# AnteMarusic/Accelerating-Genomics

Measured on AMD Instinct MI355X. Metric: Smith-Waterman affine-gap score-only GCUPS (config 2: 65536 pairs 150x150 per GPU), higher is better.
Workload: dtype int16x2 lanes, int32 scores; 1 GPU; BASELINE config 2: 65536 SW pairs 150x150 per GPU, iid ACGT + 25% related, newline sentinel aligned as the reference does; pairs_per_gpu=65536, len=150, cells_counted_per_pair=22500, parallelism=pairs sharded per GPU, no collective

## Files before the change

accelerating-genomics_amd/api.py:

```python
from __future__ import annotations

import ctypes as C
import os
import subprocess

import numpy as np

_HERE = os.path.dirname(os.path.abspath(__file__))
TUNING_KNOBS = ("AGX_SW_KERNEL", "AGX_SW_TAIL_BETA", "AGX_SW_MAX_C", "AGX_SW_FORCE_C", "AGX_SW_MAX_CLASSES", "AGX_SW_WAVES_PER_CLASS",
                "AGX_SW_SORT_WAVES", "AGX_SW_ONE_LAUNCH", "AGX_SW_DNA", "AGX_SW_RISE", "AGX_SW_PERIOD", "AGX_PHMM_PLAIN_CELL", "AGX_TRACE_CREATE", "AGX_HOST_THREADS", "AGX_FANOUT", "AGX_PHMM_TAB_BUDGET", "AGX_PHMM_MAX_C",
                "AGX_PHMM_FORCE_C", "AGX_PHMM_TAIL_BETA", "AGX_PHMM_MAX_CLASSES", "AGX_PHMM_NO_LUT", "AGX_TRACE_POOL", "AGX_NO_STREAM_PRIO", "AGX_SW_I32_CLASSIC", "AGX_SW_PIECE_MB", "AGX_SW_PIECE_MIN_PAIRS", "AGX_PHMM_NO_ROWS", "AGX_PHMM_NO_TRAINS", "AGX_PHMM_LUT_ONE_LOOP", "AGX_SW_HOST_PLAN", "AGX_PHMM_NO_RING", "AGX_TRACE_CIGAR")
_DEFAULT_LIB = "libagx_tuning.so" if any(k in os.environ for k in TUNING_KNOBS) else "libagx.so"
LIB_PATH = os.environ.get("AGX_LIB_PATH", os.path.join(_HERE, _DEFAULT_LIB))

OK, E_ARG, E_NODEVICE, E_HIP, E_NOMEM, E_SYMBOL, E_LIMIT, E_IO, E_INTERNAL = 0, -1, -2, -3, -4, -5, -6, -7, -8
SW_ALIGN_ENDS, SW_ALIGN_SPANS = 1, 2
SW_ALIGN_MAX_QUERY_LEN, SW_ALIGN_MAX_TARGET_LEN = 2560, 65535
SW_MODE_LOCAL, SW_MODE_GLOBAL, SW_MODE_FIT, SW_MODE_EXTEND, SW_MODE_EXTEND_QUERY = 0, 1, 2, 3, 4
SwHit = np.dtype([("score", np.int32), ("a_begin", np.int32), ("a_end", np.int32), ("b_begin", np.int32), ("b_end", np.int32)])
SwStat = np.dtype([("matches", np.int32), ("pairs", np.int32)])
SW_STATS_MAX_QUERY_LEN = 1792
SW_CIGAR_MAX_QUERY_LEN = 2048
CIGAR_INS, CIGAR_DEL, CIGAR_EQ, CIGAR_DIFF = 1, 2, 7, 8
_CIGAR_CHARS = {CIGAR_INS: "I", CIGAR_DEL: "D", CIGAR_EQ: "=", CIGAR_DIFF: "X"}
OPT_SW_KERNEL = 1
OPT_SW_PLANNER = 2
SW_PLANNER_AUTO, SW_PLANNER_HOST, SW_PLANNER_DEVICE = 0, 1, 2
OPT_PHMM_TRAINS = 3
OPT_SW_TRACE_BYTES = 4
PHMM_TRAINS_AUTO, PHMM_TRAINS_OFF, PHMM_TRAINS_ON = 0, 1, 2
SW_KERNEL_AUTO, SW_KERNEL_INT32, SW_KERNEL_PACKED_SIGNED, SW_KERNEL_PACKED_BIASED = 0, 1, 2, 3
PHMM_F64, PHMM_F64_FMA, PHMM_F32, PHMM_F32_FMA = 0, 1, 2, 3
PHMM_GATK_PRIOR = 0x100

SYMBOLS = [
    "agx_version", "agx_last_error", "agx_device_count", "agx_device_name", "agx_ctx_create", "agx_ctx_destroy", "agx_ctx_device",
    "agx_ctx_stream", "agx_ctx_set_stream", "agx_ctx_sync", "agx_ctx_set_option", "agx_warmup_devices", "agx_host_alloc", "agx_host_free",
    "agx_ctx_timer_start", "agx_ctx_timer_stop", "agx_ctx_timer_mark", "agx_ctx_timer_elapsed",
    "agx_sw_batch_create", "agx_sw_batch_create_scored", "agx_sw_batch_create_matrix", "agx_sw_batch_launch", "agx_sw_batch_scores", "agx_sw_batch_bind_scores", "agx_sw_batch_info", "agx_sw_batch_destroy",
    "agx_sw_batch_create_align", "agx_sw_batch_hits", "agx_sw_align", "agx_sw_batch_create_align_mode", "agx_sw_align_mode",
    "agx_sw_batch_create_align_matrix", "agx_sw_align_matrix",
    "agx_sw_batch_create_align_stats", "agx_sw_batch_stats", "agx_sw_align_stats",
    "agx_sw_batch_create_align_cigar", "agx_sw_batch_cigars", "agx_sw_batch_cigar_info", "agx_sw_align_cigar",
# ... 561 lines not shown
```

accelerating-genomics_amd/csrc/agx_sw.cpp:

```cpp
#include "agx_sw.h"

#include <algorithm>
#include <cmath>
#include <memory>
#include <mutex>
#include <thread>

#include "agx_internal.h"
#include "agx_parallel.h"

namespace {

struct Tiling {
    int cls;
    int G;
};

bool positive(long n) { return n > 0; }
bool at_least_4(long n) { return n >= 4; }
inline double tail_beta_override() { static const double v = agx_knob_real(agx_tune("AGX_SW_TAIL_BETA"), -1.0); return v; }
int max_cols_per_lane() { static const int v = (int)agx_knob_int(agx_tune("AGX_SW_MAX_C"), AGX_SW_MAX_COLS_PER_LANE, at_least_4); return v; }
int force_cols_per_lane() { static const int v = (int)agx_knob_int(agx_tune("AGX_SW_FORCE_C"), 0); return v; }
int max_classes_override() { static const int v = (int)agx_knob_int(agx_tune("AGX_SW_MAX_CLASSES"), 0, positive); return v; }
int tuned_kernel()
// ... 152 lines not shown
struct agx_sw_batch {
    agx_ctx *ctx = nullptr;
    int family = 0;
    int align = 0;
    int mode = 0;
    int stats = 0;
    DevBuf lstat;
    PinBuf lstat_stage;
    int cigar = 0;
    std::vector<uint64_t> tr_goff;
    std::vector<SwWalkRec> tr_walk;
    uint64_t tr_dwords = 0, tr_slot_words = 0;
    DevBuf goff, walkrec;
    uint32_t *trace_p = nullptr;
    bool cig_valid = false;
    std::vector<agx_sw_hit> cig_hits;
    std::vector<uint64_t> cig_off;
    std::vector<uint32_t> cig_ops;
    agx_sw_cigar_info cig_info{};
    std::vector<int64_t> fix_pair;
    std::vector<int32_t> fix_score;
    agx_sw_scoring scoring{};
    DevBuf ends;
    PinBuf ends_stage;
    std::vector<uint8_t> seq;
    std::vector<uint64_t> seq_off;
    std::vector<uint32_t> seq_len;
    SwParams prm{};
    int64_t n_pairs = 0;
    DevBuf img, groups, waves, scores;
    DevBuf table;
    int rising = 0;
    bool wide = false;
    PinBuf out_stage;
    bool matrix = false;
    agx_sw_matrix mat{};
    std::vector<ClassLaunch> launches;
    agx_sw_info info{};
    struct SwPending *pending = nullptr;
    bool file_order = false;
    int32_t *bound = nullptr;
};

namespace {
int create_batch(agx_ctx *ctx, const agx_sw_scoring *scoring, const agx_sw_matrix *matrix, const uint8_t *bases,
                 const uint64_t *off, const uint32_t *len, int64_t n_pairs, agx_sw_batch **out, bool defer = false, int align = 0, int mode = 0,
                 int stats = 0, int cigar = 0);
int finish_create(agx_sw_batch *b);
void drop_pending(agx_sw_batch *b);
}

extern "C" {

void agx_sw_batch_destroy(agx_sw_batch *b)
{
    if (!b) return;
    if (b->ctx) (void)hipSetDevice(b->ctx->device);
    drop_pending(b);
    b->img.release();
    b->groups.release();
    b->waves.release();
    b->scores.release();
    b->table.release();
    b->out_stage.release();
    b->ends.release();
    b->ends_stage.release();
// ... 1014 lines not shown
                b->tr_goff[q.group0 + g] = at;
                SwWalkRec &r = b->tr_walk[pp.pair];
                r.goff = at;
                r.x_dw = x_dw[q.first + g];
                r.y_dw = y_dw[q.first + g];
                r.ca = pp.lx();
                r.cb = pp.ly;
                r.G = (uint16_t)q.G;
                r.C = (uint16_t)C;
                at += sw_trace_dwords(q.G, pp.ly, C);
            }
        b->tr_dwords = at;
        uint64_t words = 0;
        for (SwWalkRec &r : b->tr_walk) {
            r.slot = words;
            words += (uint64_t)r.ca + r.cb;
        }
        b->tr_slot_words = words;
    }
    t_records = agx_now_ms();

    }
    b->launches = launches;
    if (family == 2 && rising == 4) {
        int period = 4;
        for (int k = 0; k < kSwNumClasses; ++k)
            if ((launched_classes >> k & 1u) && kSwClasses[k] <= kSwPackedMaxShort / 64) period = std::max(period, sw_pk2_period(kSwClasses[k]));
        bool wide = period > 4 && (int64_t)bias + ((int64_t)longest_short + 1) * sc.match - prm.gf +
                                          ((int64_t)longest_long + 65 + period) * -(int64_t)prm.ge < 0x7c00;
        if (const char *e = agx_tune("AGX_SW_PERIOD")) wide = wide && !(e[0] == '4' && !e[1]);
        b->wide = wide;
        if (wide && ctx) agx_sw_pk2w_preload();
        if (trace) fprintf(stderr, "[agx_sw_batch_create] class period %d of %d\n", wide ? period : 4, period);
    }
    b->info.n_pairs = n_pairs;
    b->info.cells = cells;
    b->info.padded_cells = padded;
    b->info.input_bytes = (int64_t)(img_dw * 4 + groups_bytes + waves_bytes);
    b->info.n_launches = (int32_t)launches.size();
    b->info.n_waves = (int32_t)n_waves_total;
    b->info.planned_on_device = device_plan ? 1 : 0;
    if (!ctx) {
        if (trace)
            fprintf(stderr, "[agx_sw_batch_create, plan only] %lld pairs: pass A %.2f ms | tiling %.2f, sort %.2f, waves %.2f, records %.2f\n",
                    (long long)n_pairs, t_pass_a - t_begin, t_plan - t_pass_a, t_sort - t_plan, t_waves - t_sort, t_records - t_waves);
        *out = b;
        b = nullptr;
        done.ok = true;
        return AGX_OK;
    }

    if (uploader.joinable()) uploader.join();
    if (up_rc) {
        agx_set_error("%s", up_err);
        return up_rc;
    }
    const double t_joined = agx_now_ms();
    rc = b->img.alloc(ctx, std::max<size_t>(img_dw, 4) * 4);
    if (!rc && !device_plan) rc = b->groups.alloc(ctx, groups_bytes);
    if (!rc && !device_plan) rc = b->waves.alloc(ctx, waves_bytes);
    if (!rc && matrix) rc = b->table.alloc(ctx, table.size() * sizeof(int16_t));
    if (!rc) rc = b->scores.alloc(ctx, ((size_t)n_pairs + 1) * sizeof(int32_t));
    if (!rc) rc = b->out_stage.alloc(ctx, ((size_t)n_pairs + 1) * sizeof(int32_t));
    if (!rc && align) rc = b->ends.alloc(ctx, ((size_t)n_pairs + 1) * sizeof(uint32_t));
    if (!rc && align) rc = b->ends_stage.alloc(ctx, ((size_t)n_pairs + 1) * sizeof(uint32_t));
    if (!rc && stats == 2) rc = b->lstat.alloc(ctx, ((size_t)n_pairs + 1) * sizeof(uint32_t));
// ... 122 lines not shown
            r = agx_sw_trace_launch_class(cl.C, prm, img, (const SwGroup *)b->groups.p, wv, cl.n_waves, scores, (uint32_t *)b->ends.p, b->trace_p,
                                          (const uint64_t *)b->goff.p, st);
        else if (b->stats == 2 && b->family == 5 && b->matrix)
            r = agx_sw_anch_mat_stats_launch_class(cl.C, anch_capture, anch_flags, prm, img, (const SwGroup *)b->groups.p, wv, cl.n_waves, scores,
                                                   (uint32_t *)b->ends.p, lstat, (const int16_t *)b->table.p, st);
        else if (b->stats == 2 && b->family == 5)
            r = agx_sw_anch_stats_launch_class(cl.C, anch_capture, anch_flags, prm, img, (const SwGroup *)b->groups.p, wv, cl.n_waves, scores,
                                               (uint32_t *)b->ends.p, lstat, st);
        else if (b->stats == 2 && b->matrix)
            r = agx_sw_loc_mat_stats_launch_class(cl.C, prm, img, (const SwGroup *)b->groups.p, wv, cl.n_waves, scores, (uint32_t *)b->ends.p, lstat,
                                                  (const int16_t *)b->table.p, st);
        else if (b->stats == 2)
            r = agx_sw_loc_stats_launch_class(cl.C, prm, img, (const SwGroup *)b->groups.p, wv, cl.n_waves, scores, (uint32_t *)b->ends.p, lstat, st);
        else if (b->family == 5 && b->matrix)
            r = agx_sw_anch_mat_launch_class(cl.C, anch_capture, anch_flags, prm, img, (const SwGroup *)b->groups.p, wv, cl.n_waves, scores,
                                             (uint32_t *)b->ends.p, (const int16_t *)b->table.p, st);
        else if (b->family == 5)
            r = agx_sw_anch_launch_class(cl.C, anch_capture, anch_flags, prm, img, (const SwGroup *)b->groups.p, wv, cl.n_waves, scores,
                                         (uint32_t *)b->ends.p, st);
        else if (b->align && b->matrix)
            r = agx_sw_loc_mat_launch_class(cl.C, prm, img, (const SwGroup *)b->groups.p, wv, cl.n_waves, scores, (uint32_t *)b->ends.p,
                                            (const int16_t *)b->table.p, st);
        else if (b->align)
            r = agx_sw_loc_launch_class(cl.C, prm, img, (const SwGroup *)b->groups.p, wv, cl.n_waves, scores, (uint32_t *)b->ends.p, st);
        else if (b->matrix)
            r = agx_sw_mat_launch_class(cl.C, prm, img, (const SwGroup *)b->groups.p, wv, cl.n_waves, scores,
                                        (const int16_t *)b->table.p, st);
        else if (b->family == 3)
            r = cl.C == 0 ? agx_sw_i32d_launch_any(prm, img, (const SwGroup2 *)b->groups.p, wv, cl.n_waves, scores, st)
                          : agx_sw_i32d_launch_class(cl.C, prm, img, (const SwGroup2 *)b->groups.p, wv, cl.n_waves, scores, st);
        else if (b->family == 2 && cl.C == 0)
            r = agx_sw_pk2_launch_any(b->rising, b->wide, prm, img, (const SwGroup2 *)b->groups.p, wv, cl.n_waves, scores, st);
        else if (b->family == 2)
            r = agx_sw_pk2_launch_class(cl.C, b->rising, b->wide, prm, img, (const SwGroup2 *)b->groups.p, wv, cl.n_waves, scores, st);
        else if (b->family == 1)
            r = agx_sw_pk_launch_class(cl.C, prm, img, (const SwGroup2 *)b->groups.p, wv, cl.n_waves, scores, st);
        else
            r = (cl.C > 40 ? agx_sw_wide_launch_class : agx_sw_launch_class)(cl.C, prm, img, (const SwGroup *)b->groups.p, wv,
                                                                             cl.n_waves, scores, st);
        if (r) {
            agx_set_error("sw_fill<%d> launch failed: %s", cl.C, hipGetErrorString(hipGetLastError()));
            return AGX_E_HIP;
        }
    }
    return fan.end();
}

int agx_sw_batch_scores(agx_sw_batch *b, int32_t *scores)
{
    if (!b || (!scores && b->n_pairs)) {
        agx_set_error("agx_sw_batch_scores: null argument");
        return AGX_E_ARG;
    }
    if (!b->ctx) {
        agx_set_error("this batch was planned without a context (no device): it has no scores");
        return AGX_E_NODEVICE;
    }
    int rc = agx_bind(b->ctx);
    if (rc) return rc;
    if (b->pending) {
        rc = finish_create(b);
        if (rc) return rc;
    }
    if (b->n_pairs == 0) {
        AGX_HIP(hipStreamSynchronize(b->ctx->stream));
        return AGX_OK;
    }
// ... 838 lines not shown
```

accelerating-genomics_amd/csrc/agx_sw.h:

```cpp
#pragma once
#include <hip/hip_runtime.h>

#include <algorithm>
#include <cstdint>

#include "../../include/agx.h"

struct SwGroup {
    uint32_t x_dw;
    uint32_t y_dw;
    uint32_t lx_ly;
    uint32_t out;
};

struct SwParams {
    int32_t ge;
    int32_t gf;
    int32_t hd;
    int32_t delta;
    int32_t shift;
    uint32_t ge2, gf2, hd2, delta2;
    uint32_t age2, agf2, bias2;
    uint32_t n_out;
};
// ... 7 lines not shown

struct SwWave {
    uint32_t first_group;
    uint16_t n_groups;
    uint16_t G;
    uint32_t steps;
    uint32_t reserved;
};

#define AGX_SW_FOR_EACH_CLASS(X) \
    X(4) X(6) X(8) X(10) X(12) X(14) X(16) X(18) X(20) X(22) X(24) X(26) X(28) X(30) X(32) X(34) X(36) X(38) X(40)
#define AGX_SW_FOR_EACH_WIDE_CLASS(X) X(80) X(120) X(160)
static const int kSwClasses[] = {4, 6, 8, 10, 12, 14, 16, 18, 20, 22, 24, 26, 28, 30, 32, 34, 36, 38, 40, 80, 120, 160};
static const int kSwPackedMaxShort = 64 * 40;
static const int kSwNumClasses = sizeof(kSwClasses) / sizeof(kSwClasses[0]);
static const double kSwClassCost[] = {1.373, 1.250, 1.178, 1.138, 1.112, 1.080, 1.051, 1.033, 1.025, 1.022, 1.014, 1.014, 1.011, 1.007, 1.007, 1.004, 1.004, 1.004, 1.000, 1.6, 2.2, 4.0};
static const double kSwPkClassCost[] = {1.543, 1.358, 1.278, 1.210, 1.173, 1.136, 1.111, 1.086, 1.068, 1.037, 1.025, 1.025, 1.019, 1.012, 1.006, 1.006, 1.006, 1.000, 1.000, 0, 0, 0};
static const double kSwPk2ClassCost[] = {1.851, 1.581, 1.450, 1.367, 1.318, 1.263, 1.196, 1.184, 1.145, 1.097, 1.095, 1.056, 1.049, 1.053, 1.025, 1.023, 1.022, 1.016, 1.000, 0, 0, 0};

static const double kSwI32dClassCost[] = {1.373, 1.250, 1.178, 1.138, 1.112, 1.080, 1.051, 1.033, 1.025, 1.022, 1.014, 1.014, 1.011, 1.007, 1.007, 1.004, 1.004, 1.004, 1.000, 0, 0, 0};

constexpr int kSwMatDim = 33;
int agx_sw_mat_launch_class(int cols_per_lane, const SwParams &prm, const uint32_t *img, const SwGroup *groups,
                            const SwWave *waves, uint32_t n_waves, int32_t *scores, const int16_t *table, hipStream_t s);
int agx_sw_pack_launch(bool matrix, int slots, const uint8_t *raw, const uint64_t *off, uint64_t base, const void *groups,
                       uint32_t n_groups, uint32_t n_pairs, uint32_t *img, const uint8_t *code, uint32_t *flag, int n_cu,
                       hipStream_t s);
int agx_sw_pack_dna_launch(const uint8_t *raw, const uint64_t *off, uint64_t base, void *groups, void *waves, uint32_t n_waves,
                           uint32_t n_pairs, uint32_t *img, uint32_t *flag, int n_cu, hipStream_t s);
int agx_sw_pk_launch_class(int cols_per_lane, const SwParams &prm, const uint32_t *img, const SwGroup2 *groups,
                           const SwWave *waves, uint32_t n_waves, int32_t *scores, hipStream_t s);
#define AGX_SW_PK2_KEEP_NARROW(C) (false)
constexpr int sw_pk2_period(int C) { return C >= 14 && !AGX_SW_PK2_KEEP_NARROW(C) ? C / 2 : 4; }
int agx_sw_pk2_launch_class(int cols_per_lane, int rising, bool wide, const SwParams &prm, const uint32_t *img, const SwGroup2 *groups,
                            const SwWave *waves, uint32_t n_waves, int32_t *scores, hipStream_t s);
int agx_sw_pk2w_launch_class(int cols_per_lane, const SwParams &prm, const uint32_t *img, const SwGroup2 *groups, const SwWave *waves,
                             uint32_t n_waves, int32_t *scores, hipStream_t s);
int agx_sw_pk2w_launch_any(const SwParams &prm, const uint32_t *img, const SwGroup2 *groups, const SwWave *waves, uint32_t n_waves,
                           int32_t *scores, hipStream_t s);
void agx_sw_pk2w_preload();
void agx_sw_pk2_preload();
void agx_sw_pack_preload();
void agx_sw_i32_preload();
int agx_sw_pk2_launch_any(int rising, bool wide, const SwParams &prm, const uint32_t *img, const SwGroup2 *groups, const SwWave *waves,
                          uint32_t n_waves, int32_t *scores, hipStream_t s);
int agx_sw_i32d_launch_any(const SwParams &prm, const uint32_t *img, const SwGroup2 *groups, const SwWave *waves, uint32_t n_waves, int32_t *scores,
                           hipStream_t s);
int agx_sw_i32d_launch_class(int cols_per_lane, const SwParams &prm, const uint32_t *img, const SwGroup2 *groups, const SwWave *waves,
                             uint32_t n_waves, int32_t *scores, hipStream_t s);
void agx_sw_i32d_preload();
int agx_sw_launch_class(int cols_per_lane, const SwParams &prm, const uint32_t *img, const SwGroup *groups,
                        const SwWave *waves, uint32_t n_waves, int32_t *scores, hipStream_t s);
int agx_sw_wide_launch_class(int cols_per_lane, const SwParams &prm, const uint32_t *img, const SwGroup *groups,
                             const SwWave *waves, uint32_t n_waves, int32_t *scores, hipStream_t s);
constexpr int kSwLocColBits = 12;
int agx_sw_loc_launch_class(int cols_per_lane, const SwParams &prm, const uint32_t *img, const SwGroup *groups, const SwWave *waves,
                            uint32_t n_waves, int32_t *scores, uint32_t *ends, hipStream_t s);
void agx_sw_loc_preload();
int agx_sw_anch_launch_class(int cols_per_lane, int capture, int flags, const SwParams &prm, const uint32_t *img, const SwGroup *groups,
                             const SwWave *waves, uint32_t n_waves, int32_t *scores, uint32_t *ends, hipStream_t s);
void agx_sw_anch_preload();
int agx_sw_loc_mat_launch_class(int cols_per_lane, const SwParams &prm, const uint32_t *img, const SwGroup *groups, const SwWave *waves,
                                uint32_t n_waves, int32_t *scores, uint32_t *ends, const int16_t *table, hipStream_t s);
void agx_sw_loc_mat_preload();
int agx_sw_anch_mat_launch_class(int cols_per_lane, int capture, int flags, const SwParams &prm, const uint32_t *img, const SwGroup *groups,
                                 const SwWave *waves, uint32_t n_waves, int32_t *scores, uint32_t *ends, const int16_t *table, hipStream_t s);
void agx_sw_anch_mat_preload();
#define AGX_SW_FOR_EACH_STATS_CLASS(X) X(4) X(6) X(8) X(10) X(12) X(14) X(16) X(18) X(20) X(22) X(24) X(26) X(28)
// ... 69 lines not shown
```

accelerating-genomics_amd/csrc/agx_sw_pk2_kernel.hip:

```cpp
#include "agx_sw_pk2_kernel.inc"

namespace {

template <int C, int KC>
__global__ void __launch_bounds__(256) sw_fill_pk2(const SwParams prm, const uint32_t *__restrict__ img,
                                                   const SwGroup2 *__restrict__ groups,
                                                   const SwWave *__restrict__ waves, uint32_t n_waves,
                                                   int32_t *__restrict__ scores)
{
    const uint32_t wave = __builtin_amdgcn_readfirstlane(blockIdx.x * 4u + (threadIdx.x >> 6));
    if (wave >= n_waves) return;
    pk2_body<C, KC>(prm, img, groups, waves[wave], scores);
}

template <int KC>
__global__ void __launch_bounds__(256) sw_fill_pk2_any(const SwParams prm, const uint32_t *__restrict__ img,
                                                       const SwGroup2 *__restrict__ groups,
                                                       const SwWave *__restrict__ waves, uint32_t n_waves,
                                                       int32_t *__restrict__ scores)
{
    const uint32_t wave = __builtin_amdgcn_readfirstlane(blockIdx.x * 4u + (threadIdx.x >> 6));
    if (wave >= n_waves) return;
    const SwWave w = waves[wave];
    switch (__builtin_amdgcn_readfirstlane(w.reserved) & 0xffffu) {
// ... 1 lines not shown
    case CC: pk2_body<CC, KC>(prm, img, groups, w, scores); break;
        AGX_SW_FOR_EACH_CLASS(AGX_SW_CASE)
#undef AGX_SW_CASE
    default: break;
    }
}

template <int C, int KC>
int launch(const SwParams &prm, const uint32_t *img, const SwGroup2 *groups, const SwWave *waves, uint32_t n_waves,
           int32_t *scores, hipStream_t s)
{
    const uint32_t blocks = (n_waves + 3) / 4;
    hipLaunchKernelGGL((sw_fill_pk2<C, KC>), dim3(blocks), dim3(256), 0, s, prm, img, groups, waves, n_waves, scores);
    return hipGetLastError() == hipSuccess ? 0 : -1;
}

}

int agx_sw_pk2_launch_any(int rising, bool wide, const SwParams &prm, const uint32_t *img, const SwGroup2 *groups, const SwWave *waves,
                          uint32_t n_waves, int32_t *scores, hipStream_t s)
{
    if (n_waves == 0) return 0;
    if (rising == 4 && wide) return agx_sw_pk2w_launch_any(prm, img, groups, waves, n_waves, scores, s);
    const uint32_t blocks = (n_waves + 3) / 4;
    if (rising == 4)
        hipLaunchKernelGGL(sw_fill_pk2_any<4>, dim3(blocks), dim3(256), 0, s, prm, img, groups, waves, n_waves, scores);
    else if (rising)
        hipLaunchKernelGGL(sw_fill_pk2_any<1>, dim3(blocks), dim3(256), 0, s, prm, img, groups, waves, n_waves, scores);
    else
        hipLaunchKernelGGL(sw_fill_pk2_any<0>, dim3(blocks), dim3(256), 0, s, prm, img, groups, waves, n_waves, scores);
    return hipGetLastError() == hipSuccess ? 0 : -1;
}

int agx_sw_pk2_launch_class(int cols_per_lane, int rising, bool wide, const SwParams &prm, const uint32_t *img, const SwGroup2 *groups,
                            const SwWave *waves, uint32_t n_waves, int32_t *scores, hipStream_t s)
{
    if (n_waves == 0) return 0;
    if (rising == 4 && wide && sw_pk2_period(cols_per_lane) > 4)
        return agx_sw_pk2w_launch_class(cols_per_lane, prm, img, groups, waves, n_waves, scores, s);
    switch (cols_per_lane) {
#define AGX_SW_CASE(CC) \
    case CC: return rising == 4 ? launch<CC, 4>(prm, img, groups, waves, n_waves, scores, s) : rising ? launch<CC, 1>(prm, img, groups, waves, n_waves, scores, s) : launch<CC, 0>(prm, img, groups, waves, n_waves, scores, s);
        AGX_SW_FOR_EACH_CLASS(AGX_SW_CASE)
#undef AGX_SW_CASE
    default: return -2;
    }
}

void agx_sw_pk2_preload()
{
    hipFuncAttributes a;
    (void)hipFuncGetAttributes(&a, reinterpret_cast<const void *>(&sw_fill_pk2_any<4>));
}
```

accelerating-genomics_amd/csrc/agx_sw_pk2_kernel.inc:

```
#include "agx_sw.h"
#include <type_traits>

namespace {

typedef unsigned short u16x2 __attribute__((ext_vector_type(2)));

__device__ __forceinline__ u16x2 as_v(uint32_t v) { return __builtin_bit_cast(u16x2, v); }
__device__ __forceinline__ uint32_t as_u(u16x2 v) { return __builtin_bit_cast(uint32_t, v); }
__device__ __forceinline__ uint32_t umax2(uint32_t a, uint32_t b) { return as_u(__builtin_elementwise_max(as_v(a), as_v(b))); }
__device__ __forceinline__ uint32_t umin2(uint32_t a, uint32_t b) { return as_u(__builtin_elementwise_min(as_v(a), as_v(b))); }
typedef _Float16 f16x2 __attribute__((ext_vector_type(2)));
__device__ __forceinline__ uint32_t umax3(uint32_t a, uint32_t b, uint32_t c)
{
    const f16x2 x = __builtin_bit_cast(f16x2, a), y = __builtin_bit_cast(f16x2, b), z = __builtin_bit_cast(f16x2, c);
    return __builtin_bit_cast(uint32_t, __builtin_elementwise_maximum(__builtin_elementwise_maximum(x, y), z));
}
__device__ __forceinline__ uint32_t in_vgpr(uint32_t s)
{
    uint32_t r;
    asm volatile("v_mov_b32 %0, %1" : "=v"(r) : "s"(s));
    return r;
}

#define AGX_DPP_TAKE " wave_shr:1 row_mask:0xf bank_mask:0xf bound_ctrl:0\n"
// ... 7 lines not shown
        : "=&v"(zl), "=&v"(fl), "+v"(ta), "+v"(tb), "=&v"(ma), "=&v"(mb)                                                     \
        : "v"(rowsA), "v"(rowsB), "v"(kv), "s"(start_mask), "v"(z_last), "v"(f_last), "v"(z0v)                               \
        : "vcc")

template <int K>
__device__ __forceinline__ void fast_head(uint32_t &zl, uint32_t &fl, uint32_t &ta, uint32_t &tb, uint32_t rowsA, uint32_t rowsB,
                                          uint32_t kv, uint64_t start_mask, uint32_t z_last, uint32_t f_last, uint32_t z0v)
{
    uint32_t ma, mb;
    if constexpr (K == 1)
        AGX_FAST_HEAD("BYTE_1");
    else if constexpr (K == 2)
        AGX_FAST_HEAD("BYTE_2");
    else if constexpr (K == 3)
        AGX_FAST_HEAD("BYTE_3");
    else
        AGX_FAST_HEAD("BYTE_0");
}

__device__ __forceinline__ void bytes_head(uint32_t &zl, uint32_t &fl, uint32_t &yc, uint32_t rowsA, uint32_t rowsB, uint32_t sel,
                                           uint32_t sh_sym, uint64_t start_mask, uint32_t z_last, uint32_t f_last, uint32_t z0v)
{
    uint32_t fresh;
    asm("v_perm_b32 %3, %5, %4, %6\n"
        "v_lshlrev_b32 %3, %7, %3\n"
        "s_mov_b64 vcc, %8\n"
        "v_cndmask_b32_dpp %0, %9, %11, vcc" AGX_DPP_TAKE "v_cndmask_b32_dpp %1, %10, %11, vcc" AGX_DPP_TAKE
        "v_cndmask_b32_dpp %2, %2, %3, vcc" AGX_DPP_TAKE
        : "=&v"(zl), "=&v"(fl), "+v"(yc), "=&v"(fresh)
        : "v"(rowsA), "v"(rowsB), "s"(sel), "v"(sh_sym), "s"(start_mask), "v"(z_last), "v"(f_last), "v"(z0v)
        : "vcc");
}

template <int C, bool FAST, int KC, bool WIDE = false>
__device__ __forceinline__ void pk2_fill(const SwParams &prm, const uint32_t *__restrict__ img, const SwGroup2 &g, const SwWave &w,
                                         int32_t *__restrict__ scores, int lane, int G, int gl, bool active, bool start, bool feeder)
{
    constexpr int XW = (C + 3) / 4;
    constexpr bool RISE = KC > 0;
    constexpr int NK = KC > 1 ? (WIDE ? C / 2 : KC) : 1;
    constexpr int kEnd = KC > 1 ? (C - 1) % NK : 0;
    constexpr int NM = KC > 1 ? NK + 3 : NK;
    const uint32_t sh_sym = prm.shift;
    const uint32_t col_pad = 0x100u << sh_sym;
    const uint32_t ge = in_vgpr(prm.age2), gf = in_vgpr(RISE ? prm.agf2 - prm.age2 : prm.agf2);
    const uint32_t hd = in_vgpr(FAST ? prm.hd2 - prm.delta2 : prm.hd2);
    const uint32_t bias = prm.bias2, delta = prm.delta2;
    const uint32_t z0 = prm.bias2 - prm.agf2;
    const uint32_t hd0 = in_vgpr((FAST ? prm.hd2 - prm.delta2 : prm.hd2) + (RISE ? prm.age2 : 0u));
    const uint32_t hdw = in_vgpr((FAST ? prm.hd2 - prm.delta2 : prm.hd2) + prm.age2 - (uint32_t)NK * prm.age2);
    const uint32_t ge_wrap = in_vgpr((uint32_t)NK * prm.age2), c_end = in_vgpr((uint32_t)kEnd * prm.age2);
    const uint32_t hdf = KC > 1 && kEnd > 0 ? in_vgpr((FAST ? prm.hd2 - prm.delta2 : prm.hd2) + prm.age2 - (uint32_t)kEnd * prm.age2) : hd0;
    const uint32_t ge4 = in_vgpr(4u * prm.age2);
    uint32_t zb = (RISE ? z0 + prm.age2 : z0) + (uint32_t)kEnd * prm.age2;
    constexpr bool FQ = WIDE && KC > 1;
    constexpr int NF = FQ ? NM : NK;
    uint32_t floorv[NF];
#pragma unroll
    for (int k = 0; k < NF; ++k) floorv[k] = (RISE ? bias + prm.age2 : bias) + (uint32_t)k * prm.age2;
    const uint32_t z_init = RISE ? z0 + prm.age2 : z0;
    const uint32_t kv = in_vgpr((prm.delta2 & 0xffu) << 24);
    const uint64_t start_mask = __ballot(start);
    const uint32_t lx_mask = FAST ? 0xfffu : 0x7fffu;
    const int lxA = (int)(g.lx_ly[0] & lx_mask), lxB = (int)(g.lx_ly[1] & lx_mask);
    const int lyA = (int)(g.lx_ly[0] >> 16), lyB = (int)(g.lx_ly[1] >> 16);

    const uint32_t no_row = FAST ? 0x1f1f1f1fu : 0u;
    const uint32_t *ybA = lyA > 0 ? img + g.y_dw[0] : img, *ybB = lyB > 0 ? img + g.y_dw[1] : img;
    const uint32_t lastA = lyA > 0 ? (uint32_t)((lyA + 3) >> 2) - 1u : 0u, lastB = lyB > 0 ? (uint32_t)((lyB + 3) >> 2) - 1u : 0u;
    const int nqA = feeder ? (lyA + 3) >> 2 : 0, nqB = feeder ? (lyB + 3) >> 2 : 0;
    auto loadA = [&](int q) -> uint32_t { return ybA[min((uint32_t)q, lastA)]; };
    auto loadB = [&](int q) -> uint32_t { return ybB[min((uint32_t)q, lastB)]; };
    auto row_selA = [&](int q, uint32_t v) -> uint32_t { return q < nqA ? v : no_row; };
    auto row_selB = [&](int q, uint32_t v) -> uint32_t { return q < nqB ? v : no_row; };

    uint32_t xq[C];
    constexpr int PF = C < 8 ? 2 : 1;
    uint32_t nextA[PF], nextB[PF];
    {
        const uint32_t o = (uint32_t)gl * C, d0 = o >> 2, sh = o & 3u;
        const uint32_t fillA = (FAST && !(active && g.x_dw[0])) ? 0x0c0c0c0cu : 0u;
        const uint32_t fillB = (FAST && !(active && g.x_dw[1])) ? 0x0c0c0c0cu : 0u;
        uint32_t ra[XW + 1], rb[XW + 1];
#pragma unroll
        for (int k = 0; k <= XW; ++k) {
            ra[k] = img[g.x_dw[0] + d0 + k];
            rb[k] = img[g.x_dw[1] + d0 + k];
        }
#pragma unroll
// ... 35 lines not shown
        z[j] = z_init + (uint32_t)(j % NK) * prm.age2;
        e[j] = bias + (uint32_t)(j % NK) * prm.age2;
    }
    uint32_t z_last = z_init + (uint32_t)kEnd * prm.age2, f_last = z_last, diag_in = z0 + (uint32_t)kEnd * prm.age2;
    uint32_t best[NM];
#pragma unroll
    for (int k = 0; k < NM; ++k) best[k] = z_init + (uint32_t)(KC > 1 ? k + 1 : k) * prm.age2;
    uint32_t yc = 0;
    uint32_t ta = 0, tb = 0;

    const bool last = active && gl == G - 1;
    const bool nlA = FAST && last && ((g.lx_ly[0] >> 13) & 1u), nlB = FAST && last && ((g.lx_ly[1] >> 13) & 1u);
    const int capA_t = (nlA && lxA > 0 && lyA > 0) ? lyA + G - 2 : -1, capB_t = (nlB && lxB > 0 && lyB > 0) ? lyB + G - 2 : -1;
    uint32_t cornerA = z_init + (uint32_t)kEnd * prm.age2, cornerB = cornerA;

    const int steps = (int)w.steps;
    uint32_t rowsA = 0, rowsB = 0;
    int t = 0;

    auto take_max = [&](auto sc) __attribute__((always_inline)) {
        constexpr int S = decltype(sc)::value;
#pragma unroll
        for (int k = 0; k < NK; ++k) {
#pragma unroll
            for (int j = k; j < C; j += 2 * NK) {
                if (j + NK < C)
                    best[S + k] = umax3(best[S + k], z[j], z[j + NK]);
                else
                    best[S + k] = umax2(best[S + k], z[j]);
            }
        }
    };

    auto step = [&](auto kc, auto sc, auto cc) __attribute__((always_inline)) {
        constexpr int K = decltype(kc)::value;
        constexpr int S = decltype(sc)::value;
        constexpr bool CAP = decltype(cc)::value;
        uint32_t zl, fl;
        if constexpr (FAST)
            fast_head<K>(zl, fl, ta, tb, rowsA, rowsB, kv, start_mask, z_last, f_last, zb);
        else
            bytes_head(zl, fl, yc, rowsA, rowsB, 0x0c040c00u + 0x00010001u * K, sh_sym, start_mask, z_last, f_last, zb);
        if constexpr (KC > 1 && S > 0 && S < 4)
            take_max(std::integral_constant<int, S - 1>{});
        else if constexpr (KC <= 1 && RISE)
            best[0] += ge;
        uint32_t zd = diag_in;
        diag_in = zl;
        uint32_t zleft = zl, f = fl;
#pragma unroll
        for (int j = 0; j < C; ++j) {
            const bool wrap = KC > 1 && j > 0 && j % NK == 0;
            const uint32_t up = z[j];
            uint32_t ev;
            if constexpr (RISE) {
                ev = umax3(up, e[j], floorv[(FQ && S < 4 ? S : 0) + j % NK]);
                f = umax2(zleft, f);
                if (KC == 1 && j > 0) f -= ge;
                if (KC > 1 && kEnd > 0 && j == 0) f -= c_end;
                if (wrap) f -= ge_wrap;
            } else {
                ev = umax3(up, e[j] - ge, bias);
                f = umax2(zleft, f - ge);
            }
            const uint32_t hdc = KC > 1 ? (wrap ? hdw : j ? hd0 : hdf) : (j ? hd : hd0);
            uint32_t u;
            if constexpr (FAST)
                u = (zd + hdc) + __builtin_amdgcn_perm(tb, ta, xq[j]);
            else
                u = (zd + hdc) - umin2(xq[j] ^ yc, delta);
            const uint32_t v = umax3(ev, f, u);
            const uint32_t zn = v - gf;
            e[j] = ev;
            z[j] = zn;
            zd = up;
            zleft = zn;
        }
        if constexpr (KC <= 1) {
#pragma unroll
            for (int j = 0; j < C; j += 2) best[0] = umax3(best[0], z[j], z[j + 1]);
        } else if constexpr (S >= 3)
            take_max(std::integral_constant<int, S == 3 ? 3 : 0>{});
        if constexpr (FAST && CAP) {
            cornerA = t == capA_t ? zleft : cornerA;
            cornerB = t == capB_t ? zleft : cornerB;
        }
        z_last = zleft;
        f_last = f;
        if constexpr (RISE) {
            if constexpr (!FQ || S == 4) {
#pragma unroll
                for (int k = 0; k < NF; ++k) floorv[k] += prm.age2;
            }
            zb += prm.age2;
        }
        ++t;
    };

    auto rise4 = [&]() __attribute__((always_inline)) {
        if constexpr (KC > 1) {
#pragma unroll
            for (int m = 0; m < NM; ++m) best[m] += ge4;
        }
        if constexpr (FQ) {
#pragma unroll
            for (int m = 0; m < NF; ++m) floorv[m] += 4u * prm.age2;
        }
    };
    auto quad_of_steps = [&](auto cc) __attribute__((always_inline)) {
        step(std::integral_constant<int, 0>{}, std::integral_constant<int, 0>{}, cc);
        step(std::integral_constant<int, 1>{}, std::integral_constant<int, 1>{}, cc);
        step(std::integral_constant<int, 2>{}, std::integral_constant<int, 2>{}, cc);
        step(std::integral_constant<int, 3>{}, std::integral_constant<int, 3>{}, cc);
        rise4();
    };
    auto take = [&](int q, int r) __attribute__((always_inline)) {
        rowsA = row_selA(q, nextA[r]);
        rowsB = row_selB(q, nextB[r]);
        nextA[r] = loadA(q + PF);
        nextB[r] = loadB(q + PF);
        if constexpr (WIDE) __builtin_amdgcn_sched_barrier(0);
    };
    const int quads = steps >> 2;
    int cap_first = 0x7fffffff;
    if constexpr (FAST) {
        cap_first = min(capA_t < 0 ? 0x7fffffff : capA_t, capB_t < 0 ? 0x7fffffff : capB_t);
        for (int o = 32; o > 0; o >>= 1) cap_first = min(cap_first, __shfl_xor(cap_first, o));
        cap_first = __builtin_amdgcn_readfirstlane(cap_first);
    }
    const int quads_free = min(quads, cap_first >> 2);
    constexpr std::integral_constant<bool, false> no_cap{};
    constexpr std::integral_constant<bool, FAST> cap{};
    int q = 0;
    if constexpr (PF == 1) {
        if constexpr (FAST) {
            for (; q < quads_free; ++q) {
                take(q, 0);
                quad_of_steps(no_cap);
            }
        }
        for (; q < quads; ++q) {
            take(q, 0);
            quad_of_steps(cap);
        }
    } else {
        if constexpr (FAST) {
            for (; q + 1 < quads_free; q += 2) {
                take(q, 0);
                quad_of_steps(no_cap);
                take(q + 1, 1);
                quad_of_steps(no_cap);
            }
        }
        for (; q + 1 < quads; q += 2) {
            take(q, 0);
            quad_of_steps(cap);
            take(q + 1, 1);
            quad_of_steps(cap);
        }
        if (q < quads) {
            rowsA = row_selA(q, nextA[0]);
            rowsB = row_selB(q, nextB[0]);
            quad_of_steps(cap);
            ++q;
            nextA[0] = nextA[1];
            nextB[0] = nextB[1];
        }
    }
    rowsA = row_selA(q, nextA[0]);
    rowsB = row_selB(q, nextB[0]);
#pragma unroll 1
    while (t < steps) {
        step(std::integral_constant<int, 0>{}, std::integral_constant<int, 4>{}, cap);
        rowsA >>= 8;
        rowsB >>= 8;
        if constexpr (KC > 1) {
            const uint32_t b0 = best[0];
#pragma unroll
            for (int m = 0; m + 1 < NM; ++m) best[m] = best[m + 1];
            best[NM - 1] = b0 + (uint32_t)NM * prm.age2;
        }
    }
    if constexpr (KC > 1) {
#pragma unroll
        for (int m = 0; m + 1 < NM; ++m) best[NM - 1] = umax2(best[NM - 1], best[m] + (uint32_t)(NM - 1 - m) * prm.age2);
        best[0] = best[NM - 1] - (uint32_t)NM * prm.age2;
    }

    if constexpr (FAST) {
        const uint32_t match2 = prm.hd2 - prm.agf2;
        const uint32_t ge1 = RISE ? prm.age2 & 0xffffu : 0u;
        const uint32_t off_end = (uint32_t)kEnd * (prm.age2 & 0xffffu);
        uint32_t cand = best[0];
        if (nlA) cand = (cand & 0xffff0000u) | ((cornerA + match2 + (uint32_t)(steps - 1 - capA_t) * ge1 - off_end) & 0xffffu);
        if (nlB) cand = (cand & 0xffffu) | ((cornerB + match2 + (((uint32_t)(steps - 1 - capB_t) * ge1 - off_end) << 16)) & 0xffff0000u);
        best[0] = umax2(best[0], cand);
    }
    uint32_t bestv = best[0];
    for (int o = 1; o < G; o <<= 1) {
        const uint32_t other = (uint32_t)__shfl_down((int)bestv, o);
        if (gl + o < G) bestv = umax2(bestv, other);
    }
    {
        const int off = (int)(z0 & 0xffffu) + (RISE ? (steps + 1) * (int)(prm.age2 & 0xffffu) : 0);
        const int src = (lane * G) & 63;
        const int sa = __shfl((int)(bestv & 0xffffu) - off, src), sb = __shfl((int)(bestv >> 16) - off, src);
        const uint32_t oa = (uint32_t)__shfl((int)g.out[0], src), ob = (uint32_t)__shfl((int)g.out[1], src);
        if (lane < (int)w.n_groups) {
            if (ob == oa + 1u && !(oa & 1u) && ob < prm.n_out)
                *reinterpret_cast<int2 *>(scores + oa) = make_int2(sa, sb);
            else {
                scores[oa] = sa;
                if (ob < prm.n_out) scores[ob] = sb;
            }
        }
    }
}

template <int C, int KC, bool WIDE = false>
__device__ __forceinline__ void pk2_body(const SwParams &prm, const uint32_t *__restrict__ img, const SwGroup2 *__restrict__ groups,
                                         const SwWave w, int32_t *__restrict__ scores)
{
    static_assert(C % 2 == 0, "the running maximum takes two columns per instruction");
    constexpr int KCC = KC > 1 && C < 14 ? 1 : KC;
    constexpr bool W = WIDE && KCC > 1 && sw_pk2_period(C) > 4;
    const int lane = threadIdx.x & 63;
    const int G = w.G;
    const int grp = lane / G;
    const int gl = lane - grp * G;
    const bool active = grp < (int)w.n_groups;
    const bool start = gl == 0;
    const bool feeder = active && start;

    SwGroup2 g = groups[w.first_group + (active ? grp : 0)];
    __builtin_amdgcn_s_waitcnt(0x0f70);
    __builtin_amdgcn_sched_barrier(0);
#pragma unroll
    for (int k = 0; k < 2; ++k) {
        g.x_dw[k] = active ? g.x_dw[k] : 0u;
        g.y_dw[k] = active ? g.y_dw[k] : 0u;
        g.lx_ly[k] = active ? g.lx_ly[k] : 0u;
        g.out[k] = active ? g.out[k] : 0u;
    }
    if (__builtin_amdgcn_readfirstlane(w.reserved >> 16) & 1u)
        pk2_fill<C, true, KCC, W>(prm, img, g, w, scores, lane, G, gl, active, start, feeder);
    else
        pk2_fill<C, false, KCC, W>(prm, img, g, w, scores, lane, G, gl, active, start, feeder);
}

}
```

Baseline: 9183 GCUPS.

## Add eight-step trip variant of wide pk2 kernel for long column classes

```diff
diff --git a/accelerating-genomics_amd/api.py b/accelerating-genomics_amd/api.py
--- a/accelerating-genomics_amd/api.py
+++ b/accelerating-genomics_amd/api.py
@@ -8,7 +8,7 @@
 
 _HERE = os.path.dirname(os.path.abspath(__file__))
 TUNING_KNOBS = ("AGX_SW_KERNEL", "AGX_SW_TAIL_BETA", "AGX_SW_MAX_C", "AGX_SW_FORCE_C", "AGX_SW_MAX_CLASSES", "AGX_SW_WAVES_PER_CLASS",
-                "AGX_SW_SORT_WAVES", "AGX_SW_ONE_LAUNCH", "AGX_SW_DNA", "AGX_SW_RISE", "AGX_SW_PERIOD", "AGX_PHMM_PLAIN_CELL", "AGX_TRACE_CREATE", "AGX_HOST_THREADS", "AGX_FANOUT", "AGX_PHMM_TAB_BUDGET", "AGX_PHMM_MAX_C",
+                "AGX_SW_SORT_WAVES", "AGX_SW_ONE_LAUNCH", "AGX_SW_DNA", "AGX_SW_RISE", "AGX_SW_PERIOD", "AGX_SW_TRIP", "AGX_PHMM_PLAIN_CELL", "AGX_TRACE_CREATE", "AGX_HOST_THREADS", "AGX_FANOUT", "AGX_PHMM_TAB_BUDGET", "AGX_PHMM_MAX_C",
                 "AGX_PHMM_FORCE_C", "AGX_PHMM_TAIL_BETA", "AGX_PHMM_MAX_CLASSES", "AGX_PHMM_NO_LUT", "AGX_TRACE_POOL", "AGX_NO_STREAM_PRIO", "AGX_SW_I32_CLASSIC", "AGX_SW_PIECE_MB", "AGX_SW_PIECE_MIN_PAIRS", "AGX_PHMM_NO_ROWS", "AGX_PHMM_NO_TRAINS", "AGX_PHMM_LUT_ONE_LOOP", "AGX_SW_HOST_PLAN", "AGX_PHMM_NO_RING", "AGX_TRACE_CIGAR")
 _DEFAULT_LIB = "libagx_tuning.so" if any(k in os.environ for k in TUNING_KNOBS) else "libagx.so"
 LIB_PATH = os.environ.get("AGX_LIB_PATH", os.path.join(_HERE, _DEFAULT_LIB))
diff --git a/accelerating-genomics_amd/csrc/agx_sw.cpp b/accelerating-genomics_amd/csrc/agx_sw.cpp
--- a/accelerating-genomics_amd/csrc/agx_sw.cpp
+++ b/accelerating-genomics_amd/csrc/agx_sw.cpp
@@ -208,6 +208,7 @@
     DevBuf table;
     int rising = 0;
     bool wide = false;
+    int trip = 4;
     PinBuf out_stage;
     bool matrix = false;
     agx_sw_matrix mat{};
@@ -1288,6 +1289,14 @@
         b->wide = wide;
         if (wide && ctx) agx_sw_pk2w_preload();
         if (trace) fprintf(stderr, "[agx_sw_batch_create] class period %d of %d\n", wide ? period : 4, period);
+        bool some_long = false;
+        for (const ClassLaunch &cl : launches) some_long = some_long || (cl.C > 0 && cl.C <= kSwPackedMaxShort / 64 && sw_pk2_trip(cl.C) == 8);
+        bool long_trip = wide && some_long && (int64_t)bias + ((int64_t)longest_short + 1) * sc.match - prm.gf +
+                                                      ((int64_t)longest_long + 69 + period) * -(int64_t)prm.ge < 0x7c00;
+        if (const char *e = agx_tune("AGX_SW_TRIP")) long_trip = long_trip && !(e[0] == '4' && !e[1]);
+        b->trip = long_trip ? 8 : 4;
+        if (long_trip && ctx) agx_sw_pk2l_preload();
+        if (trace) fprintf(stderr, "[agx_sw_batch_create] class trip %d\n", b->trip);
     }
     b->info.n_pairs = n_pairs;
     b->info.cells = cells;
@@ -1476,7 +1485,7 @@
         else if (b->family == 2 && cl.C == 0)
             r = agx_sw_pk2_launch_any(b->rising, b->wide, prm, img, (const SwGroup2 *)b->groups.p, wv, cl.n_waves, scores, st);
         else if (b->family == 2)
-            r = agx_sw_pk2_launch_class(cl.C, b->rising, b->wide, prm, img, (const SwGroup2 *)b->groups.p, wv, cl.n_waves, scores, st);
+            r = agx_sw_pk2_launch_class(cl.C, b->rising, b->wide, b->trip, prm, img, (const SwGroup2 *)b->groups.p, wv, cl.n_waves, scores, st);
         else if (b->family == 1)
             r = agx_sw_pk_launch_class(cl.C, prm, img, (const SwGroup2 *)b->groups.p, wv, cl.n_waves, scores, st);
         else
diff --git a/accelerating-genomics_amd/csrc/agx_sw.h b/accelerating-genomics_amd/csrc/agx_sw.h
--- a/accelerating-genomics_amd/csrc/agx_sw.h
+++ b/accelerating-genomics_amd/csrc/agx_sw.h
@@ -63,8 +63,13 @@
                            const SwWave *waves, uint32_t n_waves, int32_t *scores, hipStream_t s);
 #define AGX_SW_PK2_KEEP_NARROW(C) (false)
 constexpr int sw_pk2_period(int C) { return C >= 14 && !AGX_SW_PK2_KEEP_NARROW(C) ? C / 2 : 4; }
-int agx_sw_pk2_launch_class(int cols_per_lane, int rising, bool wide, const SwParams &prm, const uint32_t *img, const SwGroup2 *groups,
+#define AGX_SW_PK2_KEEP_QUAD(C) (false)
+constexpr int sw_pk2_trip(int C) { return sw_pk2_period(C) > 4 && !AGX_SW_PK2_KEEP_QUAD(C) ? 8 : 4; }
+int agx_sw_pk2_launch_class(int cols_per_lane, int rising, bool wide, int trip, const SwParams &prm, const uint32_t *img, const SwGroup2 *groups,
                             const SwWave *waves, uint32_t n_waves, int32_t *scores, hipStream_t s);
+int agx_sw_pk2l_launch_class(int cols_per_lane, const SwParams &prm, const uint32_t *img, const SwGroup2 *groups, const SwWave *waves,
+                             uint32_t n_waves, int32_t *scores, hipStream_t s);
+void agx_sw_pk2l_preload();
 int agx_sw_pk2w_launch_class(int cols_per_lane, const SwParams &prm, const uint32_t *img, const SwGroup2 *groups, const SwWave *waves,
                              uint32_t n_waves, int32_t *scores, hipStream_t s);
 int agx_sw_pk2w_launch_any(const SwParams &prm, const uint32_t *img, const SwGroup2 *groups, const SwWave *waves, uint32_t n_waves,
diff --git a/accelerating-genomics_amd/csrc/agx_sw_pk2_kernel.hip b/accelerating-genomics_amd/csrc/agx_sw_pk2_kernel.hip
--- a/accelerating-genomics_amd/csrc/agx_sw_pk2_kernel.hip
+++ b/accelerating-genomics_amd/csrc/agx_sw_pk2_kernel.hip
@@ -57,10 +57,12 @@
     return hipGetLastError() == hipSuccess ? 0 : -1;
 }
 
-int agx_sw_pk2_launch_class(int cols_per_lane, int rising, bool wide, const SwParams &prm, const uint32_t *img, const SwGroup2 *groups,
+int agx_sw_pk2_launch_class(int cols_per_lane, int rising, bool wide, int trip, const SwParams &prm, const uint32_t *img, const SwGroup2 *groups,
                             const SwWave *waves, uint32_t n_waves, int32_t *scores, hipStream_t s)
 {
     if (n_waves == 0) return 0;
+    if (rising == 4 && wide && trip == 8 && sw_pk2_trip(cols_per_lane) == 8)
+        return agx_sw_pk2l_launch_class(cols_per_lane, prm, img, groups, waves, n_waves, scores, s);
     if (rising == 4 && wide && sw_pk2_period(cols_per_lane) > 4)
         return agx_sw_pk2w_launch_class(cols_per_lane, prm, img, groups, waves, n_waves, scores, s);
     switch (cols_per_lane) {
diff --git a/accelerating-genomics_amd/csrc/agx_sw_pk2_kernel.inc b/accelerating-genomics_amd/csrc/agx_sw_pk2_kernel.inc
--- a/accelerating-genomics_amd/csrc/agx_sw_pk2_kernel.inc
+++ b/accelerating-genomics_amd/csrc/agx_sw_pk2_kernel.inc
@@ -63,7 +63,7 @@
         : "vcc");
 }
 
-template <int C, bool FAST, int KC, bool WIDE = false>
+template <int C, bool FAST, int KC, bool WIDE = false, int TRIP = 4>
 __device__ __forceinline__ void pk2_fill(const SwParams &prm, const uint32_t *__restrict__ img, const SwGroup2 &g, const SwWave &w,
                                          int32_t *__restrict__ scores, int lane, int G, int gl, bool active, bool start, bool feeder)
 {
@@ -71,7 +71,10 @@
     constexpr bool RISE = KC > 0;
     constexpr int NK = KC > 1 ? (WIDE ? C / 2 : KC) : 1;
     constexpr int kEnd = KC > 1 ? (C - 1) % NK : 0;
-    constexpr int NM = KC > 1 ? NK + 3 : NK;
+    constexpr bool LONG = TRIP == 8 && WIDE && KC > 1 && FAST;
+    static_assert(TRIP == 4 || LONG, "the eight-step trip exists for the DNA-coded wide column classes only");
+    constexpr int NQ = KC > 1 ? NK + 3 : NK;
+    constexpr int NM = LONG ? NK + TRIP - 1 : NQ;
     const uint32_t sh_sym = prm.shift;
     const uint32_t col_pad = 0x100u << sh_sym;
     const uint32_t ge = in_vgpr(prm.age2), gf = in_vgpr(RISE ? prm.agf2 - prm.age2 : prm.agf2);
@@ -83,9 +86,11 @@
     const uint32_t ge_wrap = in_vgpr((uint32_t)NK * prm.age2), c_end = in_vgpr((uint32_t)kEnd * prm.age2);
     const uint32_t hdf = KC > 1 && kEnd > 0 ? in_vgpr((FAST ? prm.hd2 - prm.delta2 : prm.hd2) + prm.age2 - (uint32_t)kEnd * prm.age2) : hd0;
     const uint32_t ge4 = in_vgpr(4u * prm.age2);
+    const uint32_t ge8 = LONG ? in_vgpr(8u * prm.age2) : 0u;
     uint32_t zb = (RISE ? z0 + prm.age2 : z0) + (uint32_t)kEnd * prm.age2;
     constexpr bool FQ = WIDE && KC > 1;
     constexpr int NF = FQ ? NM : NK;
+    constexpr int NFQ = FQ ? NQ : NK;
     uint32_t floorv[NF];
 #pragma unroll
     for (int k = 0; k < NF; ++k) floorv[k] = (RISE ? bias + prm.age2 : bias) + (uint32_t)k * prm.age2;
@@ -187,16 +192,18 @@
         }
     };
 
-    auto step = [&](auto kc, auto sc, auto cc) __attribute__((always_inline)) {
+    auto step = [&](auto kc, auto sc, auto cc, auto lc) __attribute__((always_inline)) {
         constexpr int K = decltype(kc)::value;
         constexpr int S = decltype(sc)::value;
         constexpr bool CAP = decltype(cc)::value;
+        constexpr int L = decltype(lc)::value;
+        static_assert(L == 4 || S < L, "the tail steps belong to the quads");
         uint32_t zl, fl;
         if constexpr (FAST)
             fast_head<K>(zl, fl, ta, tb, rowsA, rowsB, kv, start_mask, z_last, f_last, zb);
         else
             bytes_head(zl, fl, yc, rowsA, rowsB, 0x0c040c00u + 0x00010001u * K, sh_sym, start_mask, z_last, f_last, zb);
-        if constexpr (KC > 1 && S > 0 && S < 4)
+        if constexpr (KC > 1 && S > 0 && S < L)
             take_max(std::integral_constant<int, S - 1>{});
         else if constexpr (KC <= 1 && RISE)
             best[0] += ge;
@@ -209,7 +216,7 @@
             const uint32_t up = z[j];
             uint32_t ev;
             if constexpr (RISE) {
-                ev = umax3(up, e[j], floorv[(FQ && S < 4 ? S : 0) + j % NK]);
+                ev = umax3(up, e[j], floorv[(FQ && S < L ? S : 0) + j % NK]);
                 f = umax2(zleft, f);
                 if (KC == 1 && j > 0) f -= ge;
                 if (KC > 1 && kEnd > 0 && j == 0) f -= c_end;
@@ -234,8 +241,8 @@
         if constexpr (KC <= 1) {
 #pragma unroll
             for (int j = 0; j < C; j += 2) best[0] = umax3(best[0], z[j], z[j + 1]);
-        } else if constexpr (S >= 3)
-            take_max(std::integral_constant<int, S == 3 ? 3 : 0>{});
+        } else if constexpr (S >= L - 1)
+            take_max(std::integral_constant<int, S == L - 1 ? L - 1 : 0>{});
         if constexpr (FAST && CAP) {
             cornerA = t == capA_t ? zleft : cornerA;
             cornerB = t == capB_t ? zleft : cornerB;
@@ -243,9 +250,9 @@
         z_last = zleft;
         f_last = f;
         if constexpr (RISE) {
-            if constexpr (!FQ || S == 4) {
-#pragma unroll
-                for (int k = 0; k < NF; ++k) floorv[k] += prm.age2;
+            if constexpr (!FQ || (S == 4 && L == 4)) {
+#pragma unroll
+                for (int k = 0; k < NFQ; ++k) floorv[k] += prm.age2;
             }
             zb += prm.age2;
         }
@@ -255,18 +262,19 @@
     auto rise4 = [&]() __attribute__((always_inline)) {
         if constexpr (KC > 1) {
 #pragma unroll
-            for (int m = 0; m < NM; ++m) best[m] += ge4;
+            for (int m = 0; m < NQ; ++m) best[m] += ge4;
         }
         if constexpr (FQ) {
 #pragma unroll
-            for (int m = 0; m < NF; ++m) floorv[m] += 4u * prm.age2;
+            for (int m = 0; m < NFQ; ++m) floorv[m] += 4u * prm.age2;
         }
     };
+    constexpr std::integral_constant<int, 4> quad_len{};
     auto quad_of_steps = [&](auto cc) __attribute__((always_inline)) {
-        step(std::integral_constant<int, 0>{}, std::integral_constant<int, 0>{}, cc);
-        step(std::integral_constant<int, 1>{}, std::integral_constant<int, 1>{}, cc);
-        step(std::integral_constant<int, 2>{}, std::integral_constant<int, 2>{}, cc);
-        step(std::integral_constant<int, 3>{}, std::integral_constant<int, 3>{}, cc);
+        step(std::integral_constant<int, 0>{}, std::integral_constant<int, 0>{}, cc, quad_len);
+        step(std::integral_constant<int, 1>{}, std::integral_constant<int, 1>{}, cc, quad_len);
+        step(std::integral_constant<int, 2>{}, std::integral_constant<int, 2>{}, cc, quad_len);
+        step(std::integral_constant<int, 3>{}, std::integral_constant<int, 3>{}, cc, quad_len);
         rise4();
     };
     auto take = [&](int q, int r) __attribute__((always_inline)) {
@@ -287,6 +295,50 @@
     constexpr std::integral_constant<bool, false> no_cap{};
     constexpr std::integral_constant<bool, FAST> cap{};
     int q = 0;
+    if constexpr (LONG) {
+        static_assert(PF == 1, "a trip takes its two row quads through one register each");
+        constexpr std::integral_constant<int, 8> trip_len{};
+        auto half_trip = [&](auto s0) __attribute__((always_inline)) {
+            constexpr int S0 = decltype(s0)::value;
+            step(std::integral_constant<int, 0>{}, std::integral_constant<int, S0>{}, no_cap, trip_len);
+            step(std::integral_constant<int, 1>{}, std::integral_constant<int, S0 + 1>{}, no_cap, trip_len);
+            step(std::integral_constant<int, 2>{}, std::integral_constant<int, S0 + 2>{}, no_cap, trip_len);
+            step(std::integral_constant<int, 3>{}, std::integral_constant<int, S0 + 3>{}, no_cap, trip_len);
+        };
+        const uint32_t no_row_v = no_row, lastA_v = lastA;
+        auto take_apart = [&](int qq) __attribute__((always_inline)) {
+            uint32_t ia, ra, rb;
+            uint64_t ma;
+            asm("v_cmp_lt_u32 %[ma], %[q], %[na]\n"
+                "v_cmp_lt_u32 vcc, %[q], %[nb]\n"
+                "v_min_u32 %[ia], %[q1], %[la]\n"
+                "v_cndmask_b32 %[ra], %[nr], %[va], %[ma]\n"
+                "v_cndmask_b32 %[rb], %[nr], %[vb], vcc\n"
+                : [ma] "=&s"(ma), [ia] "=&v"(ia), [ra] "=&v"(ra), [rb] "=v"(rb)
+                : [q] "s"(qq), [q1] "s"(qq + 1), [na] "v"(nqA), [nb] "v"(nqB), [la] "v"(lastA_v), [nr] "v"(no_row_v),
+                  [va] "v"(nextA[0]), [vb] "v"(nextB[0])
+                : "vcc");
+            rowsA = ra;
+            rowsB = rb;
+            const uint32_t *pa = ybA + ia, *pb = ybB + min((uint32_t)(qq + 1), lastB);
+            nextA[0] = *pa;
+            nextB[0] = *pb;
+            asm volatile("" ::"v"(pa), "v"(pb));
+            __builtin_amdgcn_sched_barrier(0);
+        };
+        for (; q + 1 < quads_free; q += 2) {
+            take_apart(q);
+            half_trip(std::integral_constant<int, 0>{});
+            take_apart(q + 1);
+            half_trip(std::integral_constant<int, 4>{});
+#pragma unroll
+            for (int m = 0; m < NM; ++m) best[m] += ge8;
+#pragma unroll
+            for (int m = 0; m < NF; ++m) floorv[m] += 8u * prm.age2;
+        }
+#pragma unroll
+        for (int m = NQ; m < NM; ++m) best[NQ - 1] = umax2(best[NQ - 1], best[m] - (uint32_t)(m - NQ + 1) * prm.age2);
+    }
     if constexpr (PF == 1) {
         if constexpr (FAST) {
             for (; q < quads_free; ++q) {
@@ -326,20 +378,20 @@
     rowsB = row_selB(q, nextB[0]);
 #pragma unroll 1
     while (t < steps) {
-        step(std::integral_constant<int, 0>{}, std::integral_constant<int, 4>{}, cap);
+        step(std::integral_constant<int, 0>{}, std::integral_constant<int, 4>{}, cap, quad_len);
         rowsA >>= 8;
         rowsB >>= 8;
         if constexpr (KC > 1) {
             const uint32_t b0 = best[0];
 #pragma unroll
-            for (int m = 0; m + 1 < NM; ++m) best[m] = best[m + 1];
-            best[NM - 1] = b0 + (uint32_t)NM * prm.age2;
+            for (int m = 0; m + 1 < NQ; ++m) best[m] = best[m + 1];
+            best[NQ - 1] = b0 + (uint32_t)NQ * prm.age2;
         }
     }
     if constexpr (KC > 1) {
 #pragma unroll
-        for (int m = 0; m + 1 < NM; ++m) best[NM - 1] = umax2(best[NM - 1], best[m] + (uint32_t)(NM - 1 - m) * prm.age2);
-        best[0] = best[NM - 1] - (uint32_t)NM * prm.age2;
+        for (int m = 0; m + 1 < NQ; ++m) best[NQ - 1] = umax2(best[NQ - 1], best[m] + (uint32_t)(NQ - 1 - m) * prm.age2);
+        best[0] = best[NQ - 1] - (uint32_t)NQ * prm.age2;
     }
 
     if constexpr (FAST) {
@@ -372,7 +424,7 @@
     }
 }
 
-template <int C, int KC, bool WIDE = false>
+template <int C, int KC, bool WIDE = false, int TRIP = 4>
 __device__ __forceinline__ void pk2_body(const SwParams &prm, const uint32_t *__restrict__ img, const SwGroup2 *__restrict__ groups,
                                          const SwWave w, int32_t *__restrict__ scores)
 {
@@ -398,7 +450,7 @@
         g.out[k] = active ? g.out[k] : 0u;
     }
     if (__builtin_amdgcn_readfirstlane(w.reserved >> 16) & 1u)
-        pk2_fill<C, true, KCC, W>(prm, img, g, w, scores, lane, G, gl, active, start, feeder);
+        pk2_fill<C, true, KCC, W, W ? TRIP : 4>(prm, img, g, w, scores, lane, G, gl, active, start, feeder);
     else
         pk2_fill<C, false, KCC, W>(prm, img, g, w, scores, lane, G, gl, active, start, feeder);
 }
diff --git a/accelerating-genomics_amd/csrc/agx_sw_pk2l_kernel.hip b/accelerating-genomics_amd/csrc/agx_sw_pk2l_kernel.hip
--- /dev/null
+++ b/accelerating-genomics_amd/csrc/agx_sw_pk2l_kernel.hip
@@ -0,0 +1,48 @@
+#include "agx_sw_pk2_kernel.inc"
+
+namespace {
+
+template <int C>
+__global__ void __launch_bounds__(256) sw_fill_pk2l(const SwParams prm, const uint32_t *__restrict__ img,
+                                                    const SwGroup2 *__restrict__ groups,
+                                                    const SwWave *__restrict__ waves, uint32_t n_waves,
+                                                    int32_t *__restrict__ scores)
+{
+    const uint32_t wave = __builtin_amdgcn_readfirstlane(blockIdx.x * 4u + (threadIdx.x >> 6));
+    if (wave >= n_waves) return;
+    pk2_body<C, 4, true, 8>(prm, img, groups, waves[wave], scores);
+}
+
+template <int C>
+int launch(const SwParams &prm, const uint32_t *img, const SwGroup2 *groups, const SwWave *waves, uint32_t n_waves,
+           int32_t *scores, hipStream_t s)
+{
+    if constexpr (sw_pk2_trip(C) == 8) {
+        const uint32_t blocks = (n_waves + 3) / 4;
+        hipLaunchKernelGGL((sw_fill_pk2l<C>), dim3(blocks), dim3(256), 0, s, prm, img, groups, waves, n_waves, scores);
+        return hipGetLastError() == hipSuccess ? 0 : -1;
+    } else
+        return -2;
+}
+
+}
+
+int agx_sw_pk2l_launch_class(int cols_per_lane, const SwParams &prm, const uint32_t *img, const SwGroup2 *groups, const SwWave *waves,
+                             uint32_t n_waves, int32_t *scores, hipStream_t s)
+{
+    if (n_waves == 0) return 0;
+    switch (cols_per_lane) {
+#define AGX_SW_CASE(CC) \
+    case CC: return launch<CC>(prm, img, groups, waves, n_waves, scores, s);
+        AGX_SW_FOR_EACH_CLASS(AGX_SW_CASE)
+#undef AGX_SW_CASE
+    default: return -2;
+    }
+}
+
+void agx_sw_pk2l_preload()
+{
+    static_assert(sw_pk2_trip(38) == 8, "the headline's class is built long");
+    hipFuncAttributes a;
+    (void)hipFuncGetAttributes(&a, reinterpret_cast<const void *>(&sw_fill_pk2l<38>));
+}
```

After: 9175 GCUPS. No clear change (-0.1%).
